# Shwai-He/VLM-Compression

Measured on NVIDIA B200. Metric: s_per_vicuna7b_block_pruned, lower is better.
Workload: dtype f32

## Files before the change

vlm-compression_b200/csrc/cholesky.cu:

```cuda
#include <stdlib.h>
#include <atomic>
#include <map>
#include <mutex>
#include <utility>
#include "gemm3x.cuh"

namespace vlmc {

constexpr int kNB = 128;
constexpr int kPotrfThreads = 128;

constexpr int kFlipUnroll = 4;

__global__ void __launch_bounds__(256)
flip_copy_kernel(const float* __restrict__ H, int64_t ldh, float* __restrict__ F, int64_t ldf, int C, int flip,
                 int* __restrict__ status) {
  const int j = blockIdx.x * blockDim.x + threadIdx.x;
  if (j >= C) return;
  bool bad = false;
  const int first = j & ~127;
  for (int i0 = first + blockIdx.y; i0 < C; i0 += gridDim.y * kFlipUnroll) {
    float v[kFlipUnroll];
#pragma unroll
    for (int u = 0; u < kFlipUnroll; ++u) {
      const int i = i0 + u * (int)gridDim.y;
      if (i < C) v[u] = flip ? H[(int64_t)(C - 1 - i) * ldh + (C - 1 - j)] : H[(int64_t)i * ldh + j];
    }
#pragma unroll
    for (int u = 0; u < kFlipUnroll; ++u) {
      const int i = i0 + u * (int)gridDim.y;
      if (i < C) {
        F[(int64_t)i * ldf + j] = v[u];
        bad |= !isfinite(v[u]);
      }
    }
  }
  if (bad) atomicOr(status, (int)VLMC_NONFINITE);
}

__global__ void __launch_bounds__(256)
lower_to_upper_transpose_kernel(const float* __restrict__ L, int64_t ldl, float* __restrict__ U, int64_t ldu, int C) {
  __shared__ float tile[32][33];
  const int bi = blockIdx.y * 32, bj = blockIdx.x * 32;
  const int tx = threadIdx.x & 31, ty = threadIdx.x >> 5;
  if (bj + 31 >= bi) {
#pragma unroll
    for (int r = ty; r < 32; r += 8) {
      const int li = bj + r, lj = bi + tx;
      tile[r][tx] = (li < C && lj < C && lj <= li) ? L[(int64_t)li * ldl + lj] : 0.f;
    }
  }
  __syncthreads();
#pragma unroll
  for (int r = ty; r < 32; r += 8) {
    const int i = bi + r, j = bj + tx;
    if (i < C && j < C) U[(int64_t)i * ldu + j] = (j >= i && bj + 31 >= bi) ? tile[tx][r] : 0.f;
  }
}

constexpr float kHugeFactor = 1e15f;

__global__ void __launch_bounds__(256)
flip_to_upper_kernel(float* __restrict__ U, int64_t ldu, int C, int* __restrict__ status) {
  const int j = blockIdx.x * blockDim.x + threadIdx.x;
  bool huge = false;
  for (int i0 = blockIdx.y; i0 < C; i0 += gridDim.y * kFlipUnroll) {
    float v[kFlipUnroll];
#pragma unroll
    for (int u = 0; u < kFlipUnroll; ++u) {
      const int i = i0 + u * (int)gridDim.y;
      v[u] = (i < C && j < i) ? U[(int64_t)i * ldu + j] : 0.f;
    }
#pragma unroll
    for (int u = 0; u < kFlipUnroll; ++u) {
      const int i = i0 + u * (int)gridDim.y;
      if (i >= C) continue;
      if (j < i) {
        U[(int64_t)i * ldu + j] = 0.f;
        U[(int64_t)(C - 1 - i) * ldu + (C - 1 - j)] = v[u];
        huge |= !(fabsf(v[u]) <= kHugeFactor);
      } else if (j == i && i < (C + 1) / 2) {
        const int64_t a = (int64_t)i * ldu + i, b = (int64_t)(C - 1 - i) * ldu + (C - 1 - i);
        const float t = U[a], w = U[b];
        U[a] = w; U[b] = t;
        huge |= !(fabsf(t) <= kHugeFactor) || !(fabsf(w) <= kHugeFactor);
      }
    }
  }
  if (huge) atomicOr(status, (int)VLMC_HUGE_FACTOR);
}

constexpr int kPB = 16;
constexpr int kLdS = kNB + 1;
constexpr size_t kPotrfSmem = ((size_t)kNB * kLdS + 2 * (size_t)kNB * kNB + 2 * kPB + kNB) * sizeof(float);

constexpr int kPotrfIoThreads = 512;

__device__ __forceinline__ void potrf_bar() { asm volatile("bar.sync 1, 128;" ::: "memory"); }
constexpr int kBarDone0 = 2, kBarReady0 = 4, kBarInv0 = 6;
__device__ __forceinline__ void potrf_named_sync(int id, int count) { asm volatile("bar.sync %0, %1;" :: "r"(id), "r"(count) : "memory"); }
__device__ __forceinline__ void potrf_named_arrive(int id, int count) { asm volatile("bar.arrive %0, %1;" :: "r"(id), "r"(count) : "memory"); }

__global__ void __launch_bounds__(kPotrfIoThreads)
potrf_block_kernel(float* F, int64_t ldf, float* Li, int64_t ldi, int k0, int bs, int* status) {
  extern __shared__ __align__(16) float sm[];
  float* S = sm;
  float* St = S + kNB * kLdS;
  float* Xs = St + kNB * kNB;
  float* colbuf = Xs + kNB * kNB;
  float* invd = colbuf + 2 * kPB;
  const int t = threadIdx.x;
  {
    float4 v[8];
#pragma unroll
    for (int u = 0; u < 8; ++u) {
      const int idx = t + u * kPotrfIoThreads, i = idx >> 5, j4 = (idx & 31) * 4;
      v[u] = make_float4(0.f, 0.f, 0.f, 0.f);
      if (i < bs && j4 <= i) v[u] = *reinterpret_cast<const float4*>(F + (int64_t)(k0 + i) * ldf + k0 + j4);
    }
#pragma unroll
    for (int u = 0; u < 8; ++u) {
      const int idx = t + u * kPotrfIoThreads, i = idx >> 5, j4 = (idx & 31) * 4;
      const float e[4] = {v[u].x, v[u].y, v[u].z, v[u].w};
#pragma unroll
      for (int q = 0; q < 4; ++q) {
        const int j = j4 + q;
        S[i * kLdS + j] = (i < bs && j <= i) ? e[q] : (i == j ? 1.f : 0.f);
      }
      *reinterpret_cast<float4*>(Xs + idx * 4) = make_float4(0.f, 0.f, 0.f, 0.f);
    }
  }
  __syncthreads();

  const int grp = t >> 7, tt = t & 127;
  if (grp == 0) {
    bool bad = false;
    const int wend = (tt | 31) + 1;
#pragma unroll 1
    for (int c0 = 0; c0 < kNB; c0 += kPB) {
      const int b = c0 / kPB;
      if (b >= 2) potrf_named_sync(kBarReady0 + (b & 1), 384);
      float a[kPB];
#pragma unroll
      for (int c = 0; c < kPB; ++c) a[c] = S[tt * kLdS + c0 + c];
      if (b >= 1 && c0 < wend) {
#pragma unroll 4
        for (int k = c0 - kPB; k < c0; ++k) {
          const float lk = St[k * kNB + tt];
          const float4* rp = reinterpret_cast<const float4*>(St + k * kNB + c0);
          const float4 r0 = rp[0], r1 = rp[1], r2 = rp[2], r3 = rp[3];
          const float r[kPB] = {r0.x, r0.y, r0.z, r0.w, r1.x, r1.y, r1.z, r1.w, r2.x, r2.y, r2.z, r2.w, r3.x, r3.y, r3.z, r3.w};
#pragma unroll
          for (int c = 0; c < kPB; ++c) a[c] = fmaf(-lk, r[c], a[c]);
        }
      }
#pragma unroll
      for (int j = 0; j < kPB; ++j) {
        float* buf = colbuf + (j & 1) * kPB;
        if (tt >= c0 + j && tt < c0 + kPB) buf[tt - c0] = a[j];
        potrf_bar();
        float d = buf[j];
        if (!(d > 0.f) || !isfinite(d)) { bad = true; d = 1.f; }
        const float piv = sqrtf(d);
        const float inv = 1.f / piv;
        if (tt == c0 + j) { a[j] = piv; invd[c0 + j] = inv; }
        else a[j] *= inv;
#pragma unroll
        for (int c = j + 1; c < kPB; ++c) a[c] = fmaf(-a[j], buf[c] * inv, a[c]);
      }
#pragma unroll
      for (int c = 0; c < kPB; ++c) {
        const bool low = tt >= c0 + c;
        if (low) S[tt * kLdS + c0 + c] = a[c];
        St[(c0 + c) * kNB + tt] = low ? a[c] : 0.f;
      }
      potrf_bar();
      if (b <= kNB / kPB - 3) potrf_named_arrive(kBarDone0 + (b & 1), 384);
      potrf_named_arrive(kBarInv0 + b, 256);
    }
    if (bad && tt == 0) atomicOr(status, (int)VLMC_NOT_POSDEF);
  } else if (grp == 1 || grp == 3) {
    const int h = grp == 1 ? 0 : 1;
    const int wend = (tt | 31) + 1;
#pragma unroll 1
    for (int b = 2; b < kNB / kPB; ++b) {
      const int c0 = b * kPB, cb = c0 + 8 * h;
      potrf_named_sync(kBarDone0 + (b & 1), 384);
      if (c0 < wend) {
        float a[8];
#pragma unroll
        for (int c = 0; c < 8; ++c) a[c] = S[tt * kLdS + cb + c];
#pragma unroll 4
        for (int k = 0; k < c0 - kPB; ++k) {
          const float lk = St[k * kNB + tt];
          const float4* rp = reinterpret_cast<const float4*>(St + k * kNB + cb);
          const float4 r0 = rp[0], r1 = rp[1];
          const float r[8] = {r0.x, r0.y, r0.z, r0.w, r1.x, r1.y, r1.z, r1.w};
#pragma unroll
          for (int c = 0; c < 8; ++c) a[c] = fmaf(-lk, r[c], a[c]);
        }
#pragma unroll
        for (int c = 0; c < 8; ++c) S[tt * kLdS + cb + c] = a[c];
      }
      potrf_named_arrive(kBarReady0 + (b & 1), 384);
    }
  } else {
    const int c = tt;
    const int kbeg = (tt >> 5) * 32;
#pragma unroll 1
    for (int r0 = 0; r0 < kNB; r0 += kPB) {
      potrf_named_sync(kBarInv0 + r0 / kPB, 256);
      if (r0 < kbeg) continue;
      float acc[kPB];
#pragma unroll
      for (int r = 0; r < kPB; ++r) acc[r] = 0.f;
#pragma unroll 4
      for (int k = kbeg; k < r0; ++k) {
        const float xk = Xs[k * kNB + c];
        const float4* rp = reinterpret_cast<const float4*>(St + k * kNB + r0);
        const float4 q0 = rp[0], q1 = rp[1], q2 = rp[2], q3 = rp[3];
        const float l[kPB] = {q0.x, q0.y, q0.z, q0.w, q1.x, q1.y, q1.z, q1.w, q2.x, q2.y, q2.z, q2.w, q3.x, q3.y, q3.z, q3.w};
#pragma unroll
        for (int r = 0; r < kPB; ++r) acc[r] = fmaf(l[r], xk, acc[r]);
      }
      float x[kPB];
#pragma unroll
      for (int r = 0; r < kPB; ++r) {
        float sacc = ((r0 + r == c) ? 1.f : 0.f) - acc[r];
#pragma unroll
        for (int q = 0; q < r; ++q) sacc = fmaf(-S[(r0 + r) * kLdS + r0 + q], x[q], sacc);
        x[r] = sacc * invd[r0 + r];
      }
#pragma unroll
      for (int r = 0; r < kPB; ++r) Xs[(r0 + r) * kNB + c] = x[r];
    }
  }
  __syncthreads();
#pragma unroll
  for (int u = 0; u < 8; ++u) {
    const int idx = t + u * kPotrfIoThreads, i = idx >> 5, j4 = (idx & 31) * 4;
    if (i < bs && j4 < bs) {
      float4 lo, xo;
      float* lp = &lo.x;
      float* xp = &xo.x;
#pragma unroll
      for (int q = 0; q < 4; ++q) {
        const int j = j4 + q;
        lp[q] = S[i * kLdS + j];
        xp[q] = (j <= i) ? Xs[i * kNB + j] : 0.f;
      }
      if (j4 <= i) {
        float* fp = F + (int64_t)(k0 + i) * ldf + k0 + j4;
        if (j4 + 3 <= i) *reinterpret_cast<float4*>(fp) = lo;
        else {
#pragma unroll
          for (int q = 0; q < 4; ++q) if (j4 + q <= i) fp[q] = lp[q];
        }
      }
      *reinterpret_cast<float4*>(Li + (int64_t)(k0 + i) * ldi + k0 + j4) = xo;
    }
  }
}

__global__ void diag_prepare_kernel(float* H, int64_t ldh, int C, float percdamp, float* damp_out, uint8_t* dead_out) {
  __shared__ double red[32];
  double s = 0.0;
  for (int i = threadIdx.x; i < C; i += blockDim.x) {
    float d = H[(int64_t)i * ldh + i];
    const bool dead = d == 0.f;
    if (dead) { d = 1.f; H[(int64_t)i * ldh + i] = 1.f; }
    if (dead_out) dead_out[i] = dead ? 1 : 0;
    s += (double)d;
  }
  s = warp_sum(s);
  if ((threadIdx.x & 31) == 0) red[threadIdx.x >> 5] = s;
  __syncthreads();
  if (threadIdx.x == 0) {
    double t = 0.0;
    for (int w = 0; w < (int)(blockDim.x >> 5); ++w) t += red[w];
    *damp_out = percdamp * (float)(t / (double)C);
  }
}

__global__ void add_diag_kernel(float* H, int64_t ldh, int C, const float* damp) {
  const int i = blockIdx.x * blockDim.x + threadIdx.x;
  if (i < C) H[(int64_t)i * ldh + i] += *damp;
}

static std::atomic<int> g_chol_lookahead{-1};

bool chain_lookahead_enabled() {
  const int m = g_chol_lookahead.load();
  if (m >= 0) return m != 0;
  const char* e = getenv("VLMC_CHOL_LOOKAHEAD");
  return !(e && e[0] == '0');
}

ChainSide* chain_side_for(cudaStream_t st, int user) {
  static std::mutex mu;
  static std::map<std::pair<std::pair<int, int>, cudaStream_t>, ChainSide> sides;
  int dev = 0;
  if (cudaGetDevice(&dev) != cudaSuccess) { cudaGetLastError(); return nullptr; }
  std::lock_guard<std::mutex> lock(mu);
  auto key = std::make_pair(std::make_pair(dev, user), st);
  auto it = sides.find(key);
  if (it != sides.end()) return &it->second;
  ChainSide s;
  if (cudaStreamCreateWithFlags(&s.stream, cudaStreamNonBlocking) != cudaSuccess) { cudaGetLastError(); return nullptr; }
  if (cudaEventCreateWithFlags(&s.solved, cudaEventDisableTiming) != cudaSuccess ||
      cudaEventCreateWithFlags(&s.updated, cudaEventDisableTiming) != cudaSuccess) { cudaGetLastError(); return nullptr; }
  return &sides.emplace(key, s).first->second;
}

size_t chol_workspace_bytes(int C) {
  const int nb = (C + kNB - 1) / kNB;
  const size_t half = (size_t)((nb + 1) / 2) * kNB;
  return VLMC_WS_COUNTER_BYTES + align_up((size_t)C * C * sizeof(float), 256) + align_up(half * half * sizeof(float), 256);
}

}

extern "C" int vlmc_hessian_prepare(float* H, int C, int64_t ldh, float percdamp, float* damp_out,
                                    uint8_t* dead_out, void* stream) {
  using namespace vlmc;
  if (!H || !damp_out || C < 1 || ldh < C) return VLMC_ERR_BAD_ARG;
  if (!is_device_ptr(H) || !is_device_ptr(damp_out)) return VLMC_ERR_NOT_DEVICE;
  diag_prepare_kernel<<<1, 1024, 0, (cudaStream_t)stream>>>(H, ldh, C, percdamp, damp_out, dead_out);
  return check_launch();
}

extern "C" int vlmc_hessian_add_damp(float* H, int C, int64_t ldh, const float* damp, void* stream) {
  using namespace vlmc;
  if (!H || !damp || C < 1 || ldh < C) return VLMC_ERR_BAD_ARG;
  if (!is_device_ptr(H) || !is_device_ptr(damp)) return VLMC_ERR_NOT_DEVICE;
  add_diag_kernel<<<(C + 255) / 256, 256, 0, (cudaStream_t)stream>>>(H, ldh, C, damp);
  return check_launch();
}

extern "C" int vlmc_chol_set_lookahead(int mode) {
  if (mode < -1 || mode > 1) return VLMC_ERR_BAD_ARG;
  const int prev = vlmc::g_chol_lookahead.exchange(mode);
  return prev < 0 ? 2 : prev;
}

namespace vlmc {

static int chol_superpanel() {
  if (const char* e = getenv("VLMC_CHOL_SUPERPANEL")) {
    const int v = atoi(e);
    if (v == 1 || v == 2 || v == 4 || v == 8) return v;
  }
  return 1;
}

static int chol_lower_superpanel(float* F, int64_t ldf, float* Li, int64_t ldi, int C, int* status, cudaStream_t st, int sp,
                                 int potrf_smem) {
  const int nb = (C + kNB - 1) / kNB;
  int rc;
  ChainSide* side = chain_lookahead_enabled() && nb > 2 * sp ? chain_side_for(st, 0) : nullptr;
  bool pending_b = false;
  for (int s0 = 0; s0 < nb; s0 += sp) {
    const int s1 = s0 + sp < nb ? s0 + sp : nb;
    const int e = s1 * kNB < C ? s1 * kNB : C;
    for (int k = s0; k < s1; ++k) {
      const int k0 = k * kNB;
      const int bs = (C - k0 < kNB) ? (C - k0) : kNB;
      potrf_block_kernel<<<1, kPotrfIoThreads, potrf_smem, st>>>(F, ldf, Li, ldi, k0, bs, status);
      const int below = C - k0 - bs;
      if (below <= 0) continue;
      float* panel = F + (int64_t)(k0 + bs) * ldf + k0;
      rc = gemm3x(true, below, bs, bs, 1.f, panel, ldf, Li + (int64_t)k0 * ldi + k0, ldi, 0.f, panel, ldf, 0, 0, st);
      if (rc) return rc;
      const int cols_in = e - (k0 + bs);
      if (cols_in > 0) {
        rc = gemm3x(true, below, cols_in, bs, -1.f, panel, ldf, panel, ldf, 1.f, F + (int64_t)(k0 + bs) * ldf + (k0 + bs), ldf,
                    1, 0, st);
        if (rc) return rc;
      }
    }
    const int rows_rem = C - e;
    if (rows_rem <= 0) continue;
    const float* P = F + (int64_t)e * ldf + (int64_t)s0 * kNB;
    const int K = e - s0 * kNB;
    float* trail = F + (int64_t)e * ldf + e;
    const int next_cols = sp * kNB < rows_rem ? sp * kNB : rows_rem;
    const int rest = rows_rem - next_cols;
    if (!side || rest <= 0) {
      if (pending_b) {
        if (cudaStreamWaitEvent(st, side->updated, 0) != cudaSuccess) return check_launch();
        pending_b = false;
      }
      rc = gemm3x(true, rows_rem, rows_rem, K, -1.f, P, ldf, P, ldf, 1.f, trail, ldf, 1, 0, st);
      if (rc) return rc;
      continue;
    }
    if (cudaEventRecord(side->solved, st) != cudaSuccess) return check_launch();
    if (pending_b) {
      if (cudaStreamWaitEvent(st, side->updated, 0) != cudaSuccess) return check_launch();
      pending_b = false;
    }
    rc = gemm3x(true, rows_rem, next_cols, K, -1.f, P, ldf, P, ldf, 1.f, trail, ldf, 1, 0, st);
    if (rc) return rc;
    if (cudaStreamWaitEvent(side->stream, side->solved, 0) != cudaSuccess) return check_launch();
    const float* Prest = P + (int64_t)next_cols * ldf;
    rc = gemm3x(true, rest, rest, K, -1.f, Prest, ldf, Prest, ldf, 1.f, trail + (int64_t)next_cols * ldf + next_cols, ldf, 1, 0,
                side->stream, 0, false, kNumSMs - 1);
    if (rc) return rc;
    if (cudaEventRecord(side->updated, side->stream) != cudaSuccess) return check_launch();
    pending_b = true;
  }
  if (pending_b && cudaStreamWaitEvent(st, side->updated, 0) != cudaSuccess) return check_launch();
  return check_launch();
}

static int chol_lower_blocked(float* F, int64_t ldf, float* Li, int64_t ldi, int C, int* status, cudaStream_t st) {
  static bool attr_set = false;
  const int potrf_smem = (int)kPotrfSmem;
  if (!attr_set) {
    if (cudaFuncSetAttribute(potrf_block_kernel, cudaFuncAttributeMaxDynamicSharedMemorySize, potrf_smem) != cudaSuccess)
      return check_launch();
    attr_set = true;
  }
  const int nb = (C + kNB - 1) / kNB;
  int rc;
  const int sp = chol_superpanel();
  if (sp > 1 && nb > sp) return chol_lower_superpanel(F, ldf, Li, ldi, C, status, st, sp, potrf_smem);
  ChainSide* side = chain_lookahead_enabled() && nb > 2 ? chain_side_for(st, 0) : nullptr;
  bool pending_b = false;
  for (int k = 0; k < nb; ++k) {
    const int k0 = k * kNB;
    const int bs = (C - k0 < kNB) ? (C - k0) : kNB;
    potrf_block_kernel<<<1, kPotrfIoThreads, potrf_smem, st>>>(F, ldf, Li, ldi, k0, bs, status);
    const int below = C - k0 - bs;
    if (below > 0) {
      float* panel = F + (int64_t)(k0 + bs) * ldf + k0;
      rc = gemm3x(true, below, bs, bs, 1.f, panel, ldf, Li + (int64_t)k0 * ldi + k0, ldi, 0.f, panel, ldf, 0, 0, st);
      if (rc) return rc;
      float* trail = F + (int64_t)(k0 + bs) * ldf + (k0 + bs);
      const int bs2 = below < kNB ? below : kNB;
      if (!side) {
        rc = gemm3x(true, below, below, bs, -1.f, panel, ldf, panel, ldf, 1.f, trail, ldf, 1, 0, st);
        if (rc) return rc;
        continue;
      }
      const int rest = below - bs2;
      if (rest > 0 && cudaEventRecord(side->solved, st) != cudaSuccess) return check_launch();
      if (pending_b) {
        if (cudaStreamWaitEvent(st, side->updated, 0) != cudaSuccess) return check_launch();
        pending_b = false;
      }
      rc = gemm3x(true, below, bs2, bs, -1.f, panel, ldf, panel, ldf, 1.f, trail, ldf, 0, 0, st);
      if (rc) return rc;
      if (rest > 0) {
        if (cudaStreamWaitEvent(side->stream, side->solved, 0) != cudaSuccess) return check_launch();
        const float* prest = panel + (int64_t)bs2 * ldf;
        rc = gemm3x(true, rest, rest, bs, -1.f, prest, ldf, prest, ldf, 1.f, trail + (int64_t)bs2 * ldf + bs2, ldf, 1, 0,
                    side->stream, 0, false, kNumSMs - 1);
        if (rc) return rc;
        if (cudaEventRecord(side->updated, side->stream) != cudaSuccess) return check_launch();
        pending_b = true;
      }
    }
  }
  if (pending_b && cudaStreamWaitEvent(st, side->updated, 0) != cudaSuccess) return check_launch();
  return check_launch();
}

static int chol_arg_checks(const float* H, int C, int64_t ldh, float* U, int64_t ldu, int* status, void* ws, size_t ws_bytes) {
  if (!H || !U || !status || !ws || C < 1 || ldh < C || ldu < C) return VLMC_ERR_BAD_ARG;
  if ((C & 3) || (ldh & 3) || (ldu & 3) || ((uintptr_t)H & 15) || ((uintptr_t)U & 15)) return VLMC_ERR_UNSUPPORTED;
  if (!is_device_ptr(H) || !is_device_ptr(U) || !is_device_ptr(status) || !is_device_ptr(ws)) return VLMC_ERR_NOT_DEVICE;
  if (ws_bytes < chol_workspace_bytes(C)) return VLMC_ERR_WORKSPACE;
  return VLMC_OK;
}

}

extern "C" int vlmc_chol_inv_upper(const float* H, int C, int64_t ldh, float* U, int64_t ldu, int* status,
                                   void* ws, size_t ws_bytes, void* stream) {
  using namespace vlmc;
  int rc = chol_arg_checks(H, C, ldh, U, ldu, status, ws, ws_bytes);
  if (rc) return rc;
  cudaStream_t st = (cudaStream_t)stream;
  char* base = reinterpret_cast<char*>(ws) + VLMC_WS_COUNTER_BYTES;
  float* F = reinterpret_cast<float*>(base);
  const int64_t ldf = C;
  float* X = reinterpret_cast<float*>(base + align_up((size_t)C * C * sizeof(float), 256));
  const int nb = (C + kNB - 1) / kNB;

  if (cudaMemsetAsync(status, 0, sizeof(int), st) != cudaSuccess) return check_launch();
  if (cudaMemset2DAsync(U, ldu * sizeof(float), 0, (size_t)C * sizeof(float), C, st) != cudaSuccess) return check_launch();
  const int flip_rows = C < kNumSMs * 4 ? C : kNumSMs * 4;
  flip_copy_kernel<<<dim3((C + 255) / 256, flip_rows), 256, 0, st>>>(H, ldh, F, ldf, C, 1, status);

  rc = chol_lower_blocked(F, ldf, U, ldu, C, status, st);
  if (rc) return rc;

  int starts[512], ends[512];
  if (nb > 512) return VLMC_ERR_UNSUPPORTED;
  int nn = nb;
  for (int k = 0; k < nb; ++k) { starts[k] = k * kNB; ends[k] = (k + 1) * kNB < C ? (k + 1) * kNB : C; }
  while (nn > 1) {
    int out = 0;
    for (int q = 0; q + 1 < nn; q += 2) {
      const int a = starts[q], b = ends[q], c = ends[q + 1];
      const int m = c - b, n = b - a;
      rc = gemm3x(false, m, n, n, 1.f, F + (int64_t)b * ldf + a, ldf, U + (int64_t)a * ldu + a, ldu, 0.f, X, n, 0, 0, st, 1);
      if (rc) return rc;
      rc = gemm3x(false, m, n, m, -1.f, U + (int64_t)b * ldu + b, ldu, X, n, 0.f, U + (int64_t)b * ldu + a, ldu, 0, 0, st, 2);
      if (rc) return rc;
      starts[out] = a; ends[out] = c; ++out;
    }
    if (nn & 1) { starts[out] = starts[nn - 1]; ends[out] = ends[nn - 1]; ++out; }
    nn = out;
  }
  flip_to_upper_kernel<<<dim3((C + 255) / 256, flip_rows), 256, 0, st>>>(U, ldu, C, status);
  return check_launch();
}

extern "C" int vlmc_gram_upper(const float* U, int C, int64_t ldu, float* Hinv, int64_t ldh, void* stream) {
  using namespace vlmc;
  if (!U || !Hinv || C < 1 || ldu < C || ldh < C) return VLMC_ERR_BAD_ARG;
  if ((C & 3) || (ldu & 3) || (ldh & 3) || ((uintptr_t)U & 15) || ((uintptr_t)Hinv & 15)) return VLMC_ERR_UNSUPPORTED;
  if (!is_device_ptr(U) || !is_device_ptr(Hinv)) return VLMC_ERR_NOT_DEVICE;
  return gemm3x(false, C, C, C, 1.f, U, ldu, U, ldu, 0.f, Hinv, ldh, 0, 0, (cudaStream_t)stream, 0, true);
}

extern "C" int vlmc_chol_upper(const float* A, int C, int64_t lda, float* U, int64_t ldu, int* status,
                               void* ws, size_t ws_bytes, void* stream) {
  using namespace vlmc;
  int rc = chol_arg_checks(A, C, lda, U, ldu, status, ws, ws_bytes);
  if (rc) return rc;
  cudaStream_t st = (cudaStream_t)stream;
  float* F = reinterpret_cast<float*>(reinterpret_cast<char*>(ws) + VLMC_WS_COUNTER_BYTES);
  const int64_t ldf = C;
  if (cudaMemsetAsync(status, 0, sizeof(int), st) != cudaSuccess) return check_launch();
  const int flip_rows = C < kNumSMs * 4 ? C : kNumSMs * 4;
  flip_copy_kernel<<<dim3((C + 255) / 256, flip_rows), 256, 0, st>>>(A, lda, F, ldf, C, 0, status);
  rc = chol_lower_blocked(F, ldf, U, ldu, C, status, st);
  if (rc) return rc;
  lower_to_upper_transpose_kernel<<<dim3((C + 31) / 32, (C + 31) / 32), 256, 0, st>>>(F, ldf, U, ldu, C);
  return check_launch();
}

namespace vlmc {

__global__ void __launch_bounds__(256)
nonfinite_count_kernel(const float* __restrict__ A, int rows, int cols, int64_t lda, unsigned long long* __restrict__ out) {
  unsigned int pos = 0, neg = 0, nan = 0;
  for (int64_t idx = (int64_t)blockIdx.x * blockDim.x + threadIdx.x; idx < (int64_t)rows * cols;
       idx += (int64_t)gridDim.x * blockDim.x) {
    const float v = A[(idx / cols) * lda + (idx % cols)];
    if (isinf(v)) { if (v > 0.f) ++pos; else ++neg; }
    else if (v != v) ++nan;
  }
  if (pos) atomicAdd(out + 0, (unsigned long long)pos);
  if (neg) atomicAdd(out + 1, (unsigned long long)neg);
  if (nan) atomicAdd(out + 2, (unsigned long long)nan);
}

__global__ void __launch_bounds__(256)
replace_inf_kernel(float* __restrict__ A, int rows, int cols, int64_t lda, float value, int negative) {
  for (int64_t idx = (int64_t)blockIdx.x * blockDim.x + threadIdx.x; idx < (int64_t)rows * cols;
       idx += (int64_t)gridDim.x * blockDim.x) {
    float* p = A + (idx / cols) * lda + (idx % cols);
    const float v = *p;
    if (isinf(v) && ((v < 0.f) == (negative != 0))) *p = value;
  }
}

__global__ void diag_abs_mean_kernel(const float* A, int64_t lda, int C, float scale, float* out) {
  __shared__ double red[32];
  double s = 0.0;
  for (int i = threadIdx.x; i < C; i += blockDim.x) s += (double)fabsf(A[(int64_t)i * lda + i]);
  s = warp_sum(s);
  if ((threadIdx.x & 31) == 0) red[threadIdx.x >> 5] = s;
  __syncthreads();
  if (threadIdx.x == 0) {
    double t = 0.0;
    for (int w = 0; w < (int)(blockDim.x >> 5); ++w) t += red[w];
    *out = scale * (float)(t / (double)C);
  }
}

}

extern "C" int vlmc_matrix_nonfinite_count(const float* A, int rows, int cols, int64_t lda, unsigned long long* out3,
                                           void* stream) {
  using namespace vlmc;
  if (!A || !out3 || rows < 1 || cols < 1 || lda < cols) return VLMC_ERR_BAD_ARG;
  if (!is_device_ptr(A) || !is_device_ptr(out3)) return VLMC_ERR_NOT_DEVICE;
  cudaStream_t st = (cudaStream_t)stream;
  if (cudaMemsetAsync(out3, 0, 3 * sizeof(unsigned long long), st) != cudaSuccess) return check_launch();
  nonfinite_count_kernel<<<kNumSMs * 8, 256, 0, st>>>(A, rows, cols, lda, out3);
  return check_launch();
}

extern "C" int vlmc_matrix_replace_inf(float* A, int rows, int cols, int64_t lda, float value, int negative, void* stream) {
  using namespace vlmc;
  if (!A || rows < 1 || cols < 1 || lda < cols) return VLMC_ERR_BAD_ARG;
  if (!is_device_ptr(A)) return VLMC_ERR_NOT_DEVICE;
  replace_inf_kernel<<<kNumSMs * 8, 256, 0, (cudaStream_t)stream>>>(A, rows, cols, lda, value, negative);
  return check_launch();
}

extern "C" int vlmc_diag_abs_mean(const float* A, int C, int64_t lda, float scale, float* out, void* stream) {
  using namespace vlmc;
  if (!A || !out || C < 1 || lda < C) return VLMC_ERR_BAD_ARG;
  if (!is_device_ptr(A) || !is_device_ptr(out)) return VLMC_ERR_NOT_DEVICE;
  diag_abs_mean_kernel<<<1, 1024, 0, (cudaStream_t)stream>>>(A, lda, C, scale, out);
  return check_launch();
}
```

vlm-compression_b200/csrc/gemm3x.cu:

```cuda
#include "tc.cuh"
#include "gemm3x.cuh"

namespace vlmc {

constexpr int kG3M = 128;
constexpr int kG3K = 32;
constexpr int kG3Threads = 12 * 32;
constexpr int kG3CvtWarp0 = 2, kG3CvtWarps = 2, kG3EpiWarp0 = 4, kG3EpiWarps = 8;
constexpr uint32_t kG3ABytes = kG3M * kG3K * 4;

template <int TN> struct G3Cfg {
  static constexpr uint32_t kBBytes = TN * kG3K * 4;
  static constexpr uint32_t kStageBytes = 2 * (kG3ABytes + kBBytes);
  static constexpr int kStages = TN == 256 ? 2 : 3;
};

constexpr int kG3MaxStages = 3;
struct __align__(8) G3Barriers {
  uint64_t full[kG3MaxStages], conv[kG3MaxStages], empty[kG3MaxStages], tmem_full[2], tmem_empty[2];
  uint32_t tmem_base;
};

struct G3Params {
  float* C;
  int64_t ldc;
  int M, N, K;
  float alpha, beta;
  int tri, kc;
  int kmode;
  int nbi, nbj, ntiles;
};

__device__ __forceinline__ uint64_t g3_desc_k(uint32_t saddr) {
  uint64_t d = 0;
  d |= (uint64_t)((saddr & 0x3ffff) >> 4);
  d |= (uint64_t)1 << 16;
  d |= (uint64_t)(1024 >> 4) << 32;
  d |= (uint64_t)1 << 46;
  d |= (uint64_t)2 << 61;
  return d;
}
__device__ __forceinline__ uint64_t g3_desc_mn(uint32_t saddr) {
  uint64_t d = 0;
  d |= (uint64_t)((saddr & 0x3ffff) >> 4);
  d |= (uint64_t)((kG3K * 128) >> 4) << 16;
  d |= (uint64_t)(512 >> 4) << 32;
  d |= (uint64_t)1 << 46;
  d |= (uint64_t)1 << 61;
  return d;
}

template <int TN>
__device__ __forceinline__ void g3_tile(int t, const G3Params& p, int& bi, int& bj) {
  if (!p.tri) { bi = t / p.nbj; bj = t - bi * p.nbj; return; }
  for (bi = 0; bi < p.nbi; ++bi) {
    int cnt = (bi * kG3M + kG3M - 1) / TN + 1;
    if (cnt > p.nbj) cnt = p.nbj;
    if (t < cnt) { bj = t; return; }
    t -= cnt;
  }
  bj = 0;
}

template <int TN>
__device__ __forceinline__ void g3_krange(const G3Params& p, int bi, int bj, int nslices, int& sb, int& se) {
  sb = 0; se = nslices;
  if (p.kmode == 1) {
    sb = (bj * TN) / kG3K;
  } else if (p.kmode == 2) {
    const int e = (bi * kG3M + kG3M + kG3K - 1) / kG3K;
    if (e < se) se = e;
  }
}

__device__ __forceinline__ void g3_split(const uint4& raw, uint4& hi, uint4& lo) {
  const uint32_t r[4] = {raw.x, raw.y, raw.z, raw.w};
  uint32_t h[4], l[4];
#pragma unroll
  for (int e = 0; e < 4; ++e) {
    asm("cvt.rna.tf32.f32 %0, %1;" : "=r"(h[e]) : "f"(__uint_as_float(r[e])));
    l[e] = __float_as_uint(__fsub_rn(__uint_as_float(r[e]), __uint_as_float(h[e])));
  }
  hi = make_uint4(h[0], h[1], h[2], h[3]);
  lo = make_uint4(l[0], l[1], l[2], l[3]);
}

template <int TN, bool B_MN, bool CHUNKED, bool A_MN>
__global__ void __launch_bounds__(kG3Threads, 1)
gemm3x_kernel(const __grid_constant__ CUtensorMap amap, const __grid_constant__ CUtensorMap bmap, const G3Params p,
              const uint32_t idesc) {
  using Cfg = G3Cfg<TN>;
  constexpr int kStages = Cfg::kStages;
  constexpr uint32_t kBBytes = Cfg::kBBytes, kStageBytes = Cfg::kStageBytes;
  extern __shared__ __align__(1024) uint8_t smem_raw[];
  uint8_t* smem = reinterpret_cast<uint8_t*>((reinterpret_cast<uintptr_t>(smem_raw) + 1023) & ~(uintptr_t)1023);
  G3Barriers* bars = reinterpret_cast<G3Barriers*>(smem + kStages * kStageBytes + kG3EpiWarps * 4096);

  const int warp = threadIdx.x >> 5, lane = threadIdx.x & 31;

  if (warp == 0 && lane == 0) {
    asm volatile("prefetch.tensormap [%0];" :: "l"(&amap) : "memory");
    asm volatile("prefetch.tensormap [%0];" :: "l"(&bmap) : "memory");
    for (int s = 0; s < kStages; ++s) {
      mbar_init(&bars->full[s], 1);
      mbar_init(&bars->conv[s], kG3CvtWarps * 32);
      mbar_init(&bars->empty[s], 1);
    }
    for (int s = 0; s < 2; ++s) { mbar_init(&bars->tmem_full[s], 1); mbar_init(&bars->tmem_empty[s], kG3EpiWarps); }
    asm volatile("fence.mbarrier_init.release.cluster;" ::: "memory");
  }
  if (warp == 1) {
    asm volatile("tcgen05.alloc.cta_group::1.sync.aligned.shared::cta.b32 [%0], %1;"
                 :: "r"(smem_u32(&bars->tmem_base)), "r"((uint32_t)(2 * TN)) : "memory");
    asm volatile("tcgen05.relinquish_alloc_permit.cta_group::1.sync.aligned;" ::: "memory");
  }
  tc_fence_before();
  __syncthreads();
  tc_fence_after();
  const uint32_t tmem_base = bars->tmem_base;

  const int nslices = (p.K + kG3K - 1) / kG3K;
  const int slices_per_chunk = CHUNKED ? p.kc / kG3K : nslices;

  if (warp == 0) {
    if (lane == 0) {
      int stage = 0; uint32_t phase = 0;
      for (int t = blockIdx.x; t < p.ntiles; t += gridDim.x) {
        int bi, bj;
        g3_tile<TN>(t, p, bi, bj);
        const int m0 = bi * kG3M, n0 = bj * TN;
        int sbeg, send;
        g3_krange<TN>(p, bi, bj, nslices, sbeg, send);
        for (int ks = sbeg; ks < send; ++ks) {
          const int k0 = ks * kG3K;
          mbar_wait(&bars->empty[stage], phase ^ 1);
          uint8_t* sa = smem + stage * kStageBytes;
          uint8_t* sb = sa + 2 * kG3ABytes;
          mbar_expect_tx(&bars->full[stage], kG3ABytes + kBBytes);
          if (A_MN) {
#pragma unroll
            for (int q = 0; q < kG3M / 32; ++q) tma_load_2d(sa + q * (kG3K * 128), &amap, &bars->full[stage], m0 + q * 32, k0);
          } else {
            tma_load_2d(sa, &amap, &bars->full[stage], k0, m0);
          }
          if (B_MN) {
#pragma unroll
            for (int q = 0; q < TN / 32; ++q) tma_load_2d(sb + q * (kG3K * 128), &bmap, &bars->full[stage], n0 + q * 32, k0);
          } else {
            tma_load_2d(sb, &bmap, &bars->full[stage], k0, n0);
          }
          if (++stage == kStages) { stage = 0; phase ^= 1; }
        }
      }
    }
  } else if (warp == 1) {
    if (lane == 0) {
      int stage = 0; uint32_t phase = 0;
      int acc = 0; uint32_t acc_phase = 0;
      for (int t = blockIdx.x; t < p.ntiles; t += gridDim.x) {
        int bi, bj, tb, te;
        g3_tile<TN>(t, p, bi, bj);
        g3_krange<TN>(p, bi, bj, nslices, tb, te);
        for (int sbeg = tb; sbeg < te; sbeg += slices_per_chunk) {
          int send = sbeg + slices_per_chunk;
          if (send > te) send = te;
          mbar_wait(&bars->tmem_empty[acc], acc_phase ^ 1);
          tc_fence_after();
          const uint32_t d_tmem = tmem_base + acc * TN;
          uint32_t accumulate = 0;
          for (int ks = sbeg; ks < send; ++ks) {
            mbar_wait(&bars->conv[stage], phase);
            tc_fence_after();
            const uint32_t sa = smem_u32(smem + stage * kStageBytes);
            const uint32_t sb = sa + 2 * kG3ABytes;
#pragma unroll
            for (int kk = 0; kk < kG3K / 8; ++kk) {
              const uint64_t a_hi = A_MN ? g3_desc_mn(sa + kk * 1024) : g3_desc_k(sa + kk * 32);
              const uint64_t a_lo = A_MN ? g3_desc_mn(sa + kG3ABytes + kk * 1024) : g3_desc_k(sa + kG3ABytes + kk * 32);
              const uint64_t b_hi = B_MN ? g3_desc_mn(sb + kk * 1024) : g3_desc_k(sb + kk * 32);
              const uint64_t b_lo = B_MN ? g3_desc_mn(sb + kBBytes + kk * 1024) : g3_desc_k(sb + kBBytes + kk * 32);
              tc_mma_tf32(d_tmem, a_lo, b_hi, idesc, accumulate);
              tc_mma_tf32(d_tmem, a_hi, b_lo, idesc, 1);
              tc_mma_tf32(d_tmem, a_hi, b_hi, idesc, 1);
              accumulate = 1;
            }
            tc_commit(&bars->empty[stage]);
            if (++stage == kStages) { stage = 0; phase ^= 1; }
          }
          tc_commit(&bars->tmem_full[acc]);
          if (++acc == 2) { acc = 0; acc_phase ^= 1; }
        }
      }
    }
  } else if (warp >= kG3CvtWarp0 && warp < kG3CvtWarp0 + kG3CvtWarps) {
    const int ct = threadIdx.x - kG3CvtWarp0 * 32;
    int stage = 0; uint32_t phase = 0;
    for (int t = blockIdx.x; t < p.ntiles; t += gridDim.x) {
      int bi, bj, tb, te;
      g3_tile<TN>(t, p, bi, bj);
      g3_krange<TN>(p, bi, bj, nslices, tb, te);
      for (int ks = tb; ks < te; ++ks) {
        mbar_wait(&bars->full[stage], phase);
        uint8_t* sa = smem + stage * kStageBytes;
        uint8_t* sb = sa + 2 * kG3ABytes;
        auto convert = [&](uint8_t* base, uint32_t bytes) {
          constexpr int kCT = kG3CvtWarps * 32, kBatch = 8;
          for (int i0 = ct; i0 < (int)(bytes / 16); i0 += kCT * kBatch) {
            uint4 raw[kBatch];
#pragma unroll
            for (int u = 0; u < kBatch; ++u) raw[u] = *reinterpret_cast<const uint4*>(base + (i0 + u * kCT) * 16);
#pragma unroll
            for (int u = 0; u < kBatch; ++u) {
              uint4 hi, lo;
              g3_split(raw[u], hi, lo);
              *reinterpret_cast<uint4*>(base + (i0 + u * kCT) * 16) = hi;
              *reinterpret_cast<uint4*>(base + bytes + (i0 + u * kCT) * 16) = lo;
            }
          }
        };
        convert(sa, kG3ABytes);
        convert(sb, kBBytes);
        fence_proxy_async_smem();
        mbar_arrive(&bars->conv[stage]);
        if (++stage == kStages) { stage = 0; phase ^= 1; }
      }
    }
  } else if (warp >= kG3EpiWarp0) {
    constexpr int kCols = TN / 2;
    constexpr int kBlocks = kCols / 32;
    const int ew = warp - kG3EpiWarp0;
    const int q = warp & 3;
    const int half = ew >> 2;
    float* stg = reinterpret_cast<float*>(smem + kStages * kStageBytes) + ew * 1024;
    const int rsub = lane >> 3, jsub = lane & 7;
    int acc = 0; uint32_t acc_phase = 0;

    auto load_c = [&](float4 (&h)[8], int row0, int col0) {
#pragma unroll
      for (int i = 0; i < 8; ++i) {
        const int gi = row0 + 4 * i + rsub, gj = col0 + 4 * jsub;
        h[i] = (p.beta != 0.f && gi < p.M && gj < p.N)
                   ? *reinterpret_cast<const float4*>(p.C + (int64_t)gi * p.ldc + gj) : make_float4(0.f, 0.f, 0.f, 0.f);
      }
    };
    auto store_block = [&](const float (&v)[32], const float4 (&h)[8], int row0, int col0) {
#pragma unroll
      for (int j = 0; j < 8; ++j)
        *reinterpret_cast<float4*>(stg + lane * 32 + ((j ^ (lane & 7)) << 2)) = make_float4(v[4 * j], v[4 * j + 1], v[4 * j + 2], v[4 * j + 3]);
      __syncwarp();
#pragma unroll
      for (int i = 0; i < 8; ++i) {
        const int r = 4 * i + rsub;
        const float4 a = *reinterpret_cast<const float4*>(stg + r * 32 + ((jsub ^ (r & 7)) << 2));
        const int gi = row0 + r, gj = col0 + 4 * jsub;
        if (gi < p.M && gj < p.N) {
          float4 o;
          o.x = fmaf(p.alpha, a.x, p.beta * h[i].x); o.y = fmaf(p.alpha, a.y, p.beta * h[i].y);
          o.z = fmaf(p.alpha, a.z, p.beta * h[i].z); o.w = fmaf(p.alpha, a.w, p.beta * h[i].w);
          *reinterpret_cast<float4*>(p.C + (int64_t)gi * p.ldc + gj) = o;
        }
      }
      __syncwarp();
    };

    for (int t = blockIdx.x; t < p.ntiles; t += gridDim.x) {
      int bi, bj;
      g3_tile<TN>(t, p, bi, bj);
      const int row0 = bi * kG3M + q * 32;
      const int col0 = bj * TN + half * kCols;
      if (CHUNKED) {
        float sum[kCols];
#pragma unroll
        for (int c = 0; c < kCols; ++c) sum[c] = 0.f;
        int tb, te;
        g3_krange<TN>(p, bi, bj, nslices, tb, te);
        const int nchunks = (te - tb + slices_per_chunk - 1) / slices_per_chunk;
        for (int ch = 0; ch < nchunks; ++ch) {
          mbar_wait(&bars->tmem_full[acc], acc_phase);
          tc_fence_after();
          const uint32_t taddr = tmem_base + ((uint32_t)(q * 32) << 16) + acc * TN + half * kCols;
#pragma unroll
          for (int c4 = 0; c4 < kBlocks; ++c4) {
            uint32_t v[32];
            tc_ld32(taddr + c4 * 32, v);
            tc_wait_ld();
#pragma unroll
            for (int c = 0; c < 32; ++c) sum[c4 * 32 + c] += __uint_as_float(v[c]);
          }
          tc_fence_before();
          __syncwarp();
          if (lane == 0) mbar_arrive(&bars->tmem_empty[acc]);
          if (++acc == 2) { acc = 0; acc_phase ^= 1; }
        }
#pragma unroll
        for (int c4 = 0; c4 < kBlocks; ++c4) {
          float4 h[8];
          load_c(h, row0, col0 + c4 * 32);
          float v[32];
#pragma unroll
          for (int c = 0; c < 32; ++c) v[c] = sum[c4 * 32 + c];
          store_block(v, h, row0, col0 + c4 * 32);
        }
      } else {
        float4 h[2][8];
        load_c(h[0], row0, col0);
        mbar_wait(&bars->tmem_full[acc], acc_phase);
        tc_fence_after();
        const uint32_t taddr = tmem_base + ((uint32_t)(q * 32) << 16) + acc * TN + half * kCols;
#pragma unroll
        for (int c4 = 0; c4 < kBlocks; ++c4) {
          if (c4 + 1 < kBlocks) load_c(h[(c4 + 1) & 1], row0, col0 + (c4 + 1) * 32);
          uint32_t u[32];
          tc_ld32(taddr + c4 * 32, u);
          tc_wait_ld();
          float v[32];
#pragma unroll
          for (int c = 0; c < 32; ++c) v[c] = __uint_as_float(u[c]);
          store_block(v, h[c4 & 1], row0, col0 + c4 * 32);
        }
        tc_fence_before();
        __syncwarp();
        if (lane == 0) mbar_arrive(&bars->tmem_empty[acc]);
        if (++acc == 2) { acc = 0; acc_phase ^= 1; }
      }
    }
  }

  tc_fence_before();
  __syncthreads();
  if (warp == 1) {
    asm volatile("tcgen05.dealloc.cta_group::1.sync.aligned.b32 %0, %1;" :: "r"(tmem_base), "r"((uint32_t)(2 * TN)) : "memory");
  }
}

template <int TN> constexpr size_t g3_smem() {
  return G3Cfg<TN>::kStages * G3Cfg<TN>::kStageBytes + kG3EpiWarps * 4096 + sizeof(G3Barriers) + 1024;
}

template <int TN, bool B_MN, bool CHUNKED, bool A_MN = false>
static int g3_launch(const CUtensorMap& amap, const CUtensorMap& bmap, G3Params p, cudaStream_t st, int max_ctas = 0) {
  auto kern = gemm3x_kernel<TN, B_MN, CHUNKED, A_MN>;
  static bool attr_set = false;
  if (!attr_set) {
    if (cudaFuncSetAttribute(kern, cudaFuncAttributeMaxDynamicSharedMemorySize, (int)g3_smem<TN>()) != cudaSuccess)
      return check_launch();
    attr_set = true;
  }
  p.nbi = (p.M + kG3M - 1) / kG3M;
  p.nbj = (p.N + TN - 1) / TN;
  if (p.tri) {
    p.ntiles = 0;
    for (int bi = 0; bi < p.nbi; ++bi) {
      int cnt = (bi * kG3M + kG3M - 1) / TN + 1;
      p.ntiles += cnt < p.nbj ? cnt : p.nbj;
    }
  } else {
    p.ntiles = p.nbi * p.nbj;
  }
  const uint32_t idesc = (1u << 4) | (2u << 7) | (2u << 10) | ((A_MN ? 1u : 0u) << 15) | ((B_MN ? 1u : 0u) << 16) |
                         ((uint32_t)(TN >> 3) << 17) | ((uint32_t)(kG3M >> 4) << 24);
  const int cap = (max_ctas > 0 && max_ctas < kNumSMs) ? max_ctas : kNumSMs;
  const int grid = p.ntiles < cap ? p.ntiles : cap;
  kern<<<grid, kG3Threads, g3_smem<TN>(), st>>>(amap, bmap, p, idesc);
  return check_launch();
}

static int g3_map(CUtensorMap* map, const float* base, uint64_t inner, uint64_t outer, int64_t ld, uint32_t box_inner,
                  uint32_t box_outer, CUtensorMapSwizzle swizzle) {
  EncodeTiledFn encode = get_encode_fn();
  if (!encode) return VLMC_ERR_CUDA;
  const cuuint64_t dims[2] = {(cuuint64_t)inner, (cuuint64_t)outer};
  const cuuint64_t strides[1] = {(cuuint64_t)ld * 4};
  const cuuint32_t box[2] = {box_inner, box_outer};
  const cuuint32_t estr[2] = {1, 1};
  CUresult cr = encode(map, CU_TENSOR_MAP_DATA_TYPE_FLOAT32, 2, const_cast<float*>(base), dims, strides, box, estr,
                       CU_TENSOR_MAP_INTERLEAVE_NONE, swizzle, CU_TENSOR_MAP_L2_PROMOTION_L2_256B,
                       CU_TENSOR_MAP_FLOAT_OOB_FILL_NONE);
  if (cr != CUDA_SUCCESS) { g_last_cuda_error = (int)cr; return VLMC_ERR_CUDA; }
  return VLMC_OK;
}

int gemm3x(bool b_nk, int M, int N, int K, float alpha, const float* A, int64_t lda, const float* B, int64_t ldb,
           float beta, float* C, int64_t ldc, int tri, int kc, cudaStream_t st, int kmode, bool a_km, int max_ctas) {
  if (M <= 0 || N <= 0) return VLMC_OK;
  if (K <= 0 || !A || !B || !C) return VLMC_ERR_BAD_ARG;
  if (a_km && (b_nk || kmode != 0 || (M & 3))) return VLMC_ERR_UNSUPPORTED;
  if ((!(a_km && !b_nk) && (K & 3)) || (N & 3) || (lda & 3) || (ldb & 3) || (ldc & 3) || ((uintptr_t)A & 15) || ((uintptr_t)B & 15) ||
      ((uintptr_t)C & 15))
    return VLMC_ERR_UNSUPPORTED;
  if (kc <= 0) kc = 128;
  if (kmode < 0 || kmode > 2 || (kmode == 1 && b_nk)) return VLMC_ERR_BAD_ARG;
  kc = (kc + kG3K - 1) / kG3K * kG3K;
  const bool chunked = K > kc;
  const int TN = (!chunked && N > 128 && !a_km) ? 256 : 128;

  CUtensorMap amap, bmap;
  int rc = a_km ? g3_map(&amap, A, (uint64_t)M, (uint64_t)K, lda, 32, kG3K, CU_TENSOR_MAP_SWIZZLE_128B_ATOM_32B)
                : g3_map(&amap, A, (uint64_t)K, (uint64_t)M, lda, kG3K, kG3M, CU_TENSOR_MAP_SWIZZLE_128B);
  if (rc) return rc;
  if (b_nk) rc = g3_map(&bmap, B, (uint64_t)K, (uint64_t)N, ldb, kG3K, (uint32_t)TN, CU_TENSOR_MAP_SWIZZLE_128B);
  else rc = g3_map(&bmap, B, (uint64_t)N, (uint64_t)K, ldb, 32, kG3K, CU_TENSOR_MAP_SWIZZLE_128B_ATOM_32B);
  if (rc) return rc;

  G3Params p;
  p.C = C; p.ldc = ldc; p.M = M; p.N = N; p.K = K; p.alpha = alpha; p.beta = beta; p.tri = tri; p.kc = kc; p.kmode = kmode;
  p.nbi = p.nbj = p.ntiles = 0;
  if (a_km) {
    if (chunked) return g3_launch<128, true, true, true>(amap, bmap, p, st);
    return g3_launch<128, true, false, true>(amap, bmap, p, st);
  }
  if (chunked) return b_nk ? g3_launch<128, false, true>(amap, bmap, p, st) : g3_launch<128, true, true>(amap, bmap, p, st);
  if (TN == 256) return b_nk ? g3_launch<256, false, false>(amap, bmap, p, st, max_ctas) : g3_launch<256, true, false>(amap, bmap, p, st, max_ctas);
  return b_nk ? g3_launch<128, false, false>(amap, bmap, p, st, max_ctas) : g3_launch<128, true, false>(amap, bmap, p, st, max_ctas);
}

}

extern "C" int vlmc_gemm_tf32x3(int b_nk, int M, int N, int K, float alpha, const float* A, int64_t lda,
                                const float* B, int64_t ldb, float beta, float* C, int64_t ldc, int tri, int kc,
                                void* stream) {
  using namespace vlmc;
  if (!A || !B || !C || M < 1 || N < 1 || K < 1 || lda < K || ldc < N || ldb < (b_nk ? K : N)) return VLMC_ERR_BAD_ARG;
  if (!is_device_ptr(A) || !is_device_ptr(B) || !is_device_ptr(C)) return VLMC_ERR_NOT_DEVICE;
  return gemm3x(b_nk != 0, M, N, K, alpha, A, lda, B, ldb, beta, C, ldc, tri, kc, (cudaStream_t)stream, 0, false);
}
```

vlm-compression_b200/csrc/gemm3x.cuh:

```cuda
#pragma once
#include "common.cuh"

namespace vlmc {

int gemm3x(bool b_nk, int M, int N, int K, float alpha, const float* A, int64_t lda, const float* B, int64_t ldb,
           float beta, float* C, int64_t ldc, int tri, int kc, cudaStream_t st, int kmode = 0, bool a_km = false,
           int max_ctas = 0);

struct ChainSide { cudaStream_t stream; cudaEvent_t solved, updated; };
ChainSide* chain_side_for(cudaStream_t st, int user);
bool chain_lookahead_enabled();

}
```

Before: 0.002024.

## Batch equal-size triangular-inverse merge GEMMs into single strided launches

```diff
diff --git a/vlm-compression_b200/csrc/cholesky.cu b/vlm-compression_b200/csrc/cholesky.cu
--- a/vlm-compression_b200/csrc/cholesky.cu
+++ b/vlm-compression_b200/csrc/cholesky.cu
@@ -502,7 +502,22 @@
   for (int k = 0; k < nb; ++k) { starts[k] = k * kNB; ends[k] = (k + 1) * kNB < C ? (k + 1) * kNB : C; }
   while (nn > 1) {
     int out = 0;
-    for (int q = 0; q + 1 < nn; q += 2) {
+    const int s = ends[0] - starts[0];
+    int np = 0;
+    while (2 * np + 1 < nn && ends[2 * np] - starts[2 * np] == s && ends[2 * np + 1] - starts[2 * np + 1] == s) ++np;
+    if (np > 1 && s % kNB == 0) {
+      const int a = starts[0], b = ends[0];
+      const G3Batch b1 = {np, 2 * s, 2 * s, 2 * s, 2 * s, (int64_t)s};
+      rc = gemm3x(false, s, s, s, 1.f, F + (int64_t)b * ldf + a, ldf, U + (int64_t)a * ldu + a, ldu, 0.f, X, (int64_t)np * s,
+                  0, 0, st, 1, false, 0, &b1);
+      if (rc) return rc;
+      const G3Batch b2 = {np, 2 * s, 2 * s, 0, s, 2 * (int64_t)s * ldu + 2 * s};
+      rc = gemm3x(false, s, s, s, -1.f, U + (int64_t)b * ldu + b, ldu, X, (int64_t)np * s, 0.f, U + (int64_t)b * ldu + a, ldu,
+                  0, 0, st, 2, false, 0, &b2);
+      if (rc) return rc;
+      for (int q = 0; q < np; ++q) { starts[out] = starts[2 * q]; ends[out] = ends[2 * q + 1]; ++out; }
+    }
+    for (int q = 2 * (np > 1 && s % kNB == 0 ? np : 0); q + 1 < nn; q += 2) {
       const int a = starts[q], b = ends[q], c = ends[q + 1];
       const int m = c - b, n = b - a;
       rc = gemm3x(false, m, n, n, 1.f, F + (int64_t)b * ldf + a, ldf, U + (int64_t)a * ldu + a, ldu, 0.f, X, n, 0, 0, st, 1);
diff --git a/vlm-compression_b200/csrc/gemm3x.cu b/vlm-compression_b200/csrc/gemm3x.cu
--- a/vlm-compression_b200/csrc/gemm3x.cu
+++ b/vlm-compression_b200/csrc/gemm3x.cu
@@ -29,6 +29,9 @@
   int tri, kc;
   int kmode;
   int nbi, nbj, ntiles;
+  int tiles_per_batch;
+  int a_dm, a_dk, b_dk, b_dn;
+  int64_t c_step;
 };
 
 __device__ __forceinline__ uint64_t g3_desc_k(uint32_t saddr) {
@@ -51,7 +54,9 @@
 }
 
 template <int TN>
-__device__ __forceinline__ void g3_tile(int t, const G3Params& p, int& bi, int& bj) {
+__device__ __forceinline__ void g3_tile(int t, const G3Params& p, int& bi, int& bj, int& pb) {
+  pb = t / p.tiles_per_batch;
+  t -= pb * p.tiles_per_batch;
   if (!p.tri) { bi = t / p.nbj; bj = t - bi * p.nbj; return; }
   for (bi = 0; bi < p.nbi; ++bi) {
     int cnt = (bi * kG3M + kG3M - 1) / TN + 1;
@@ -126,28 +131,28 @@
     if (lane == 0) {
       int stage = 0; uint32_t phase = 0;
       for (int t = blockIdx.x; t < p.ntiles; t += gridDim.x) {
-        int bi, bj;
-        g3_tile<TN>(t, p, bi, bj);
-        const int m0 = bi * kG3M, n0 = bj * TN;
+        int bi, bj, pb;
+        g3_tile<TN>(t, p, bi, bj, pb);
+        const int m0 = bi * kG3M + pb * p.a_dm, n0 = bj * TN + pb * p.b_dn;
         int sbeg, send;
         g3_krange<TN>(p, bi, bj, nslices, sbeg, send);
         for (int ks = sbeg; ks < send; ++ks) {
-          const int k0 = ks * kG3K;
+          const int k0 = ks * kG3K + pb * p.a_dk, kb = ks * kG3K + pb * p.b_dk;
           mbar_wait(&bars->empty[stage], phase ^ 1);
           uint8_t* sa = smem + stage * kStageBytes;
           uint8_t* sb = sa + 2 * kG3ABytes;
           mbar_expect_tx(&bars->full[stage], kG3ABytes + kBBytes);
           if (A_MN) {
 #pragma unroll
-            for (int q = 0; q < kG3M / 32; ++q) tma_load_2d(sa + q * (kG3K * 128), &amap, &bars->full[stage], m0 + q * 32, k0);
+            for (int u = 0; u < kG3M / 32; ++u) tma_load_2d(sa + u * (kG3K * 128), &amap, &bars->full[stage], m0 + u * 32, k0);
           } else {
             tma_load_2d(sa, &amap, &bars->full[stage], k0, m0);
           }
           if (B_MN) {
 #pragma unroll
-            for (int q = 0; q < TN / 32; ++q) tma_load_2d(sb + q * (kG3K * 128), &bmap, &bars->full[stage], n0 + q * 32, k0);
+            for (int u = 0; u < TN / 32; ++u) tma_load_2d(sb + u * (kG3K * 128), &bmap, &bars->full[stage], n0 + u * 32, kb);
           } else {
-            tma_load_2d(sb, &bmap, &bars->full[stage], k0, n0);
+            tma_load_2d(sb, &bmap, &bars->full[stage], kb, n0);
           }
           if (++stage == kStages) { stage = 0; phase ^= 1; }
         }
@@ -158,8 +163,8 @@
       int stage = 0; uint32_t phase = 0;
       int acc = 0; uint32_t acc_phase = 0;
       for (int t = blockIdx.x; t < p.ntiles; t += gridDim.x) {
-        int bi, bj, tb, te;
-        g3_tile<TN>(t, p, bi, bj);
+        int bi, bj, pb, tb, te;
+        g3_tile<TN>(t, p, bi, bj, pb);
         g3_krange<TN>(p, bi, bj, nslices, tb, te);
         for (int sbeg = tb; sbeg < te; sbeg += slices_per_chunk) {
           int send = sbeg + slices_per_chunk;
@@ -196,8 +201,8 @@
     const int ct = threadIdx.x - kG3CvtWarp0 * 32;
     int stage = 0; uint32_t phase = 0;
     for (int t = blockIdx.x; t < p.ntiles; t += gridDim.x) {
-      int bi, bj, tb, te;
-      g3_tile<TN>(t, p, bi, bj);
+      int bi, bj, pb, tb, te;
+      g3_tile<TN>(t, p, bi, bj, pb);
       g3_krange<TN>(p, bi, bj, nslices, tb, te);
       for (int ks = tb; ks < te; ++ks) {
         mbar_wait(&bars->full[stage], phase);
@@ -234,13 +239,14 @@
     float* stg = reinterpret_cast<float*>(smem + kStages * kStageBytes) + ew * 1024;
     const int rsub = lane >> 3, jsub = lane & 7;
     int acc = 0; uint32_t acc_phase = 0;
+    float* cq = p.C;
 
     auto load_c = [&](float4 (&h)[8], int row0, int col0) {
 #pragma unroll
       for (int i = 0; i < 8; ++i) {
         const int gi = row0 + 4 * i + rsub, gj = col0 + 4 * jsub;
         h[i] = (p.beta != 0.f && gi < p.M && gj < p.N)
-                   ? *reinterpret_cast<const float4*>(p.C + (int64_t)gi * p.ldc + gj) : make_float4(0.f, 0.f, 0.f, 0.f);
+                   ? *reinterpret_cast<const float4*>(cq + (int64_t)gi * p.ldc + gj) : make_float4(0.f, 0.f, 0.f, 0.f);
       }
     };
     auto store_block = [&](const float (&v)[32], const float4 (&h)[8], int row0, int col0) {
@@ -257,15 +263,16 @@
           float4 o;
           o.x = fmaf(p.alpha, a.x, p.beta * h[i].x); o.y = fmaf(p.alpha, a.y, p.beta * h[i].y);
           o.z = fmaf(p.alpha, a.z, p.beta * h[i].z); o.w = fmaf(p.alpha, a.w, p.beta * h[i].w);
-          *reinterpret_cast<float4*>(p.C + (int64_t)gi * p.ldc + gj) = o;
+          *reinterpret_cast<float4*>(cq + (int64_t)gi * p.ldc + gj) = o;
         }
       }
       __syncwarp();
     };
 
     for (int t = blockIdx.x; t < p.ntiles; t += gridDim.x) {
-      int bi, bj;
-      g3_tile<TN>(t, p, bi, bj);
+      int bi, bj, pb;
+      g3_tile<TN>(t, p, bi, bj, pb);
+      cq = p.C + pb * p.c_step;
       const int row0 = bi * kG3M + q * 32;
       const int col0 = bj * TN + half * kCols;
       if (CHUNKED) {
@@ -338,7 +345,8 @@
 }
 
 template <int TN, bool B_MN, bool CHUNKED, bool A_MN = false>
-static int g3_launch(const CUtensorMap& amap, const CUtensorMap& bmap, G3Params p, cudaStream_t st, int max_ctas = 0) {
+static int g3_launch(const CUtensorMap& amap, const CUtensorMap& bmap, G3Params p, int nbatch, cudaStream_t st,
+                     int max_ctas = 0) {
   auto kern = gemm3x_kernel<TN, B_MN, CHUNKED, A_MN>;
   static bool attr_set = false;
   if (!attr_set) {
@@ -357,6 +365,8 @@
   } else {
     p.ntiles = p.nbi * p.nbj;
   }
+  p.tiles_per_batch = p.ntiles;
+  p.ntiles *= nbatch;
   const uint32_t idesc = (1u << 4) | (2u << 7) | (2u << 10) | ((A_MN ? 1u : 0u) << 15) | ((B_MN ? 1u : 0u) << 16) |
                          ((uint32_t)(TN >> 3) << 17) | ((uint32_t)(kG3M >> 4) << 24);
   const int cap = (max_ctas > 0 && max_ctas < kNumSMs) ? max_ctas : kNumSMs;
@@ -381,7 +391,8 @@
 }
 
 int gemm3x(bool b_nk, int M, int N, int K, float alpha, const float* A, int64_t lda, const float* B, int64_t ldb,
-           float beta, float* C, int64_t ldc, int tri, int kc, cudaStream_t st, int kmode, bool a_km, int max_ctas) {
+           float beta, float* C, int64_t ldc, int tri, int kc, cudaStream_t st, int kmode, bool a_km, int max_ctas,
+           const G3Batch* batch) {
   if (M <= 0 || N <= 0) return VLMC_OK;
   if (K <= 0 || !A || !B || !C) return VLMC_ERR_BAD_ARG;
   if (a_km && (b_nk || kmode != 0 || (M & 3))) return VLMC_ERR_UNSUPPORTED;
@@ -393,25 +404,33 @@
   kc = (kc + kG3K - 1) / kG3K * kG3K;
   const bool chunked = K > kc;
   const int TN = (!chunked && N > 128 && !a_km) ? 256 : 128;
+  const int nb = batch ? batch->count : 1;
+  if (nb < 1) return VLMC_ERR_BAD_ARG;
+  if (nb > 1 && (a_km || tri || (M % kG3M) || (N % TN) || (K % kG3K) || (batch->c_step & 3))) return VLMC_ERR_UNSUPPORTED;
+  const uint64_t xm = nb > 1 ? (uint64_t)(nb - 1) * batch->a_dm : 0, xak = nb > 1 ? (uint64_t)(nb - 1) * batch->a_dk : 0;
+  const uint64_t xbk = nb > 1 ? (uint64_t)(nb - 1) * batch->b_dk : 0, xn = nb > 1 ? (uint64_t)(nb - 1) * batch->b_dn : 0;
 
   CUtensorMap amap, bmap;
   int rc = a_km ? g3_map(&amap, A, (uint64_t)M, (uint64_t)K, lda, 32, kG3K, CU_TENSOR_MAP_SWIZZLE_128B_ATOM_32B)
-                : g3_map(&amap, A, (uint64_t)K, (uint64_t)M, lda, kG3K, kG3M, CU_TENSOR_MAP_SWIZZLE_128B);
+                : g3_map(&amap, A, (uint64_t)K + xak, (uint64_t)M + xm, lda, kG3K, kG3M, CU_TENSOR_MAP_SWIZZLE_128B);
   if (rc) return rc;
-  if (b_nk) rc = g3_map(&bmap, B, (uint64_t)K, (uint64_t)N, ldb, kG3K, (uint32_t)TN, CU_TENSOR_MAP_SWIZZLE_128B);
-  else rc = g3_map(&bmap, B, (uint64_t)N, (uint64_t)K, ldb, 32, kG3K, CU_TENSOR_MAP_SWIZZLE_128B_ATOM_32B);
+  if (b_nk) rc = g3_map(&bmap, B, (uint64_t)K + xbk, (uint64_t)N + xn, ldb, kG3K, (uint32_t)TN, CU_TENSOR_MAP_SWIZZLE_128B);
+  else rc = g3_map(&bmap, B, (uint64_t)N + xn, (uint64_t)K + xbk, ldb, 32, kG3K, CU_TENSOR_MAP_SWIZZLE_128B_ATOM_32B);
   if (rc) return rc;
 
   G3Params p;
   p.C = C; p.ldc = ldc; p.M = M; p.N = N; p.K = K; p.alpha = alpha; p.beta = beta; p.tri = tri; p.kc = kc; p.kmode = kmode;
-  p.nbi = p.nbj = p.ntiles = 0;
+  p.nbi = p.nbj = p.ntiles = p.tiles_per_batch = 0;
+  p.a_dm = nb > 1 ? batch->a_dm : 0; p.a_dk = nb > 1 ? batch->a_dk : 0;
+  p.b_dk = nb > 1 ? batch->b_dk : 0; p.b_dn = nb > 1 ? batch->b_dn : 0;
+  p.c_step = nb > 1 ? batch->c_step : 0;
   if (a_km) {
-    if (chunked) return g3_launch<128, true, true, true>(amap, bmap, p, st);
-    return g3_launch<128, true, false, true>(amap, bmap, p, st);
-  }
-  if (chunked) return b_nk ? g3_launch<128, false, true>(amap, bmap, p, st) : g3_launch<128, true, true>(amap, bmap, p, st);
-  if (TN == 256) return b_nk ? g3_launch<256, false, false>(amap, bmap, p, st, max_ctas) : g3_launch<256, true, false>(amap, bmap, p, st, max_ctas);
-  return b_nk ? g3_launch<128, false, false>(amap, bmap, p, st, max_ctas) : g3_launch<128, true, false>(amap, bmap, p, st, max_ctas);
+    if (chunked) return g3_launch<128, true, true, true>(amap, bmap, p, nb, st);
+    return g3_launch<128, true, false, true>(amap, bmap, p, nb, st);
+  }
+  if (chunked) return b_nk ? g3_launch<128, false, true>(amap, bmap, p, nb, st) : g3_launch<128, true, true>(amap, bmap, p, nb, st);
+  if (TN == 256) return b_nk ? g3_launch<256, false, false>(amap, bmap, p, nb, st, max_ctas) : g3_launch<256, true, false>(amap, bmap, p, nb, st, max_ctas);
+  return b_nk ? g3_launch<128, false, false>(amap, bmap, p, nb, st, max_ctas) : g3_launch<128, true, false>(amap, bmap, p, nb, st, max_ctas);
 }
 
 }
diff --git a/vlm-compression_b200/csrc/gemm3x.cuh b/vlm-compression_b200/csrc/gemm3x.cuh
--- a/vlm-compression_b200/csrc/gemm3x.cuh
+++ b/vlm-compression_b200/csrc/gemm3x.cuh
@@ -3,9 +3,10 @@
 
 namespace vlmc {
 
+struct G3Batch { int count; int a_dm, a_dk, b_dk, b_dn; int64_t c_step; };
 int gemm3x(bool b_nk, int M, int N, int K, float alpha, const float* A, int64_t lda, const float* B, int64_t ldb,
            float beta, float* C, int64_t ldc, int tri, int kc, cudaStream_t st, int kmode = 0, bool a_km = false,
-           int max_ctas = 0);
+           int max_ctas = 0, const G3Batch* batch = nullptr);
 
 struct ChainSide { cudaStream_t stream; cudaEvent_t solved, updated; };
 ChainSide* chain_side_for(cudaStream_t st, int user);
```

Measured after the change: 0.002029 (median of 6 runs). No clear change (+0.3%).
